# salesforce/gorp

Hardware: AMD Instinct MI355X
Metric: lines/sec (Gorp.extract: product-DFA match + capture offsets; results as narrow rows (int8 id + uint8 offsets, 9 B/line)) (higher is better)
Workload: dtype u8

## Files before the change

### gorp_amd/csrc/gx_api.cpp

```cpp
#include <hip/hip_runtime.h>

#include <algorithm>
#include <array>
#include <cstdio>
#include <cstddef>
#include <cstdlib>
#include <map>
#include <mutex>
#include <new>
#include <optional>
#include <string>
#include <thread>
#include <atomic>

#include "gx_by_key.hpp"
#include "gx_compile.hpp"
#include "gx_device.hpp"
#include "gx_dsl.hpp"
#include "gx_group.hpp"
#include "gx_group_quantile.hpp"
#include "gx_top_groups.hpp"
#include "gx_hop.hpp"
#include "gx_images.hpp"
#include "gx_slots.hpp"
// ... 725 lines not shown
    case 5: { GxLds L; return plan_tile_launch(I, 0, &L) ? static_cast<int64_t>(L.total_bytes) : 0; }
    case 6: { GxLds L; return plan_tile_launch(I, 0, &L) ? static_cast<int64_t>(L.nwaves) : 0; }
    case 7: return !I.tile_ok ? 0 : I.dense[0].L.tier == 3 ? 4 : I.tile_global ? 2 : I.dense[0].L.tier == 2 ? 3 : 1;
    case 8: return h->T.has_capture ? 1 : 0;
    case 10: { GxLds L; return plan_lanes_launch(I, &L, false, true) ? static_cast<int64_t>(L.nwaves) : 0; }
    case 11: { GxLds L; return plan_lanes_launch(I, &L, true, false) ? static_cast<int64_t>(L.nwaves) : 0; }
    case 12: return I.tile_ok ? static_cast<int64_t>(I.dense[0].L.table_bytes) : 0;
    case 13: return I.tile_ok ? static_cast<int64_t>(I.dense[0].L.regs_wave_bytes) : 0;
    case 14: return I.hop[0].ok ? static_cast<int64_t>(H.n_states) : 0;
    case 15: return I.hop[0].ok ? static_cast<int64_t>(H.full.n_hot) : 0;
    case 21: return I.hop[0].ok ? static_cast<int64_t>(H.small.n_hot) : 0;
    case 16: return I.hop[0].ok ? static_cast<int64_t>(H.n_reachable_hot) : 0;
    case 17: return I.hop[0].ok ? static_cast<int64_t>(H.n_chains) : 0;
    case 18: { GxLds L; return plan_hop_launch(I, 0, &L) ? static_cast<int64_t>(L.nwaves) : 0; }
    case 20: return I.hop[0].ok ? static_cast<int64_t>(H.full.n_lds_rows) : 0;
    case 22: return I.hop[1].ok ? static_cast<int64_t>(I.hop[1].img.n_states) : 0;
    case 24: return static_cast<int64_t>(h->slots.promises_broken.load());
    case 30: return static_cast<int64_t>(h->peer_image_bytes);
    case 25: return h->last_kernel.load();
    case 31: return h->last_fits.load();
    case 32: return h->last_limit.load();
    case 33: return static_cast<int64_t>(h->last_utf8_lines.load());
    case 34: return static_cast<int64_t>(h->last_utf8_units.load());
    case 26: return I.hop_reason;
    case 28: return static_cast<int64_t>(h->svc.enabled ? h->svc.launches : -1);
    case 27: { int64_t c = 0; for (auto& r : h->T.rules) c += r.pike ? 1 : 0; return c; }
    case 35: {
        if (!h->T.has_pike()) return -1;
        uint32_t lane_ints = 0, blocks = 0;
        pike_sizing(h->T, &lane_ints, &blocks);
// ... 2792 lines not shown
```

### gorp_amd/csrc/gx_hop.cpp

```cpp
#include "gx_hop.hpp"

#include <algorithm>
#include <deque>

namespace gx {

namespace {
inline bool has(const ClassSet& s, int c) { return (s[c >> 6] >> (c & 63)) & 1ull; }
inline void put(ClassSet& s, int c) { s[c >> 6] |= 1ull << (c & 63); }
}

std::vector<int> order_classes(const std::map<ClassSet, uint64_t>& weight, int ncls) {
    std::vector<std::vector<int>> blocks(1);
    for (int c = 0; c < ncls; ++c) blocks[0].push_back(c);
    std::vector<std::pair<uint64_t, ClassSet>> by_weight;
    for (auto& w : weight) {
        int size = 0;
        for (int c = 0; c < ncls; ++c) size += has(w.first, c) ? 1 : 0;
        if (size > 1 && size < ncls) by_weight.push_back({w.second * static_cast<uint64_t>(size), w.first});
    }
    std::sort(by_weight.begin(), by_weight.end(), [](const std::pair<uint64_t, ClassSet>& a, const std::pair<uint64_t, ClassSet>& b) {
        return a.first != b.first ? a.first > b.first : a.second < b.second;
    });
    for (auto& ws : by_weight) {
// ... 82 lines not shown
        for (int i = 0; i < 128; ++i) {
            if (!in_set(m, i)) continue;
            int j = i;
            long w = 0;
            while (j < 128 && in_set(m, j)) { w += byte_worth(j); ++j; }
            if (w > best.weight || (w == best.weight && j - i > best.hi - best.lo + 1)) best = Range{i, j - 1, w};
            i = j;
        }
        return best;
    };

    struct Exit { bool any = false; Range r; uint32_t entry = 0; ClassSet set{}; };
    std::vector<Range> run(S);
    std::vector<long> run_weight(S, 0);
    std::vector<std::array<uint8_t, 8>> set_table(1, std::array<uint8_t, 8>{0, 0, 0, 0, 0x80, 0x80, 0x80, 0x80});
    std::map<std::array<uint8_t, 8>, uint32_t> set_index;
    std::vector<uint32_t> set_of(S, 0);
    auto loop_set = [&](const ClassSet& cs) -> uint32_t {
        const ByteSet m = bytes_of(cs);
        std::vector<Range> rs;
        for (int i = 0; i < 128; ++i) {
            if (!in_set(m, i)) continue;
            int j = i;
            long w = 0;
            while (j < 128 && in_set(m, j)) { w += byte_worth(j); ++j; }
            rs.push_back(Range{i, j - 1, w});
            i = j;
        }
        if (rs.size() < 2) return 0u;
        std::stable_sort(rs.begin(), rs.end(), [](const Range& a, const Range& b) { return a.weight != b.weight ? a.weight > b.weight : (a.hi - a.lo) > (b.hi - b.lo); });
        if (rs.size() > 4) rs.resize(4);
        std::sort(rs.begin(), rs.end(), [](const Range& a, const Range& b) { return a.lo < b.lo; });
        std::array<uint8_t, 8> key{0, 0, 0, 0, 0x80, 0x80, 0x80, 0x80};
        for (size_t q = 0; q < rs.size(); ++q) { key[q] = static_cast<uint8_t>(rs[q].lo); key[4 + q] = static_cast<uint8_t>(0x7F - rs[q].hi); }
        auto it = set_index.find(key);
        if (it != set_index.end()) return it->second;
        if (set_table.size() >= 256) return 0u;
        set_table.push_back(key);
        set_index[key] = static_cast<uint32_t>(set_table.size() - 1);
        return static_cast<uint32_t>(set_table.size() - 1);
    };
    std::vector<Exit> exit_of(S);
    std::vector<std::vector<uint32_t>> plausible_targets(S);
    for (size_t s = 0; s < S; ++s) {
        int n_plausible = 0;
        const Group* only = nullptr;
        for (auto& g : groups[s]) {
            if (g.entry == static_cast<uint32_t>(s)) {
                run[s] = best_range(g.set);
                run_weight[s] = g.weight;
                if (s != dead) set_of[s] = loop_set(g.set);
                continue;
            }
            if (g.weight > 0) { ++n_plausible; only = &g; plausible_targets[s].push_back(g.entry & 0xFFFFu); }
        }
        if (n_plausible == 1) {
            exit_of[s].any = true;
            exit_of[s].r = best_range(only->set);
            exit_of[s].entry = only->entry;
            exit_of[s].set = only->set;
        }
    }

    struct Chain { int klen = 0, tail = -1; uint8_t lo[HOP_CHAIN], span[HOP_CHAIN]; uint32_t target = 0, col[2] = {0, 0}, off[2] = {0, 0}, tail_set = 0; };
    std::vector<Chain> chain(S);
    for (size_t s = 0; s < S; ++s) {
// ... 4 lines not shown
        for (uint32_t k = 0; k < HOP_CHAIN; ++k) {
            if (k > 0 && run_weight[cur] > 4) break;
            const Exit& x = exit_of[cur];
            if (!x.any || x.r.hi < x.r.lo) break;
            const bool ranged = x.r.hi > x.r.lo || x.r.lo == 0;
            if (ranged && ch.tail >= 0) break;
            const uint32_t col = x.entry >> 16;
            if (col) {
                if (nops == 2) break;
                ch.col[nops] = col;
                ch.off[nops] = k;
                ++nops;
            }
            if (ranged) {
                ch.tail = static_cast<int>(k);
                ch.tail_set = loop_set(x.set);
            }
            ch.lo[k] = static_cast<uint8_t>(x.r.lo);
            ch.span[k] = static_cast<uint8_t>(x.r.hi - x.r.lo);
            ch.klen = static_cast<int>(k) + 1;
            cur = x.entry & 0xFFFFu;
        }
        ch.target = static_cast<uint32_t>(cur);
    }

    std::vector<uint32_t> order;
    std::vector<char> seen(S, 0);
    std::deque<uint32_t> queue;
    auto visit = [&](uint32_t s) { if (!seen[s]) { seen[s] = 1; queue.push_back(s); } };
    visit(0);
    while (!queue.empty()) {
// ... 54 lines not shown
        const Chain& ch = chain[s];
        uint32_t run_lo = 0, run_k = 0x80;
        if (run[s].hi >= run[s].lo && s != dead) { run_lo = static_cast<uint32_t>(run[s].lo); run_k = 0x7Fu - static_cast<uint32_t>(run[s].hi); ++out.n_runs; }
        r[0] = run_lo | run_k << 8 | static_cast<uint32_t>(ch.klen) << 16 | set_of[s] << 24;
        r[1] = (ch.klen ? perm[ch.target] : 0u) | ch.off[0] << 16 | ch.off[1] << 24;
        r[2] = (ch.col[0] << 7) | (ch.col[1] << 7) << 16;
        uint8_t lits[HOP_CHAIN];
        for (uint32_t k = 0; k < HOP_CHAIN; ++k) lits[k] = (static_cast<int>(k) < ch.klen && static_cast<int>(k) != ch.tail) ? ch.lo[k] : 0;
        if (ch.tail >= 0) r[3] = static_cast<uint32_t>(ch.tail) | static_cast<uint32_t>(ch.lo[ch.tail]) << 8 | static_cast<uint32_t>(ch.span[ch.tail]) << 16 | ch.tail_set << 24;
        else r[3] = 0u | 0u << 8 | 0xFFu << 16;
        if (ch.klen == 0) r[3] = 0u | 2u << 8 | 0u << 16, lits[0] = 0x01;
        else ++out.n_chains;
        memcpy(&r[4], lits, 8);
    }

    for (size_t s = 0; s < S; ++s) {
        const uint32_t* r = &hops[s * (HOP_REC_BYTES / 4)];
        const uint32_t run_lo = r[0] & 0xFFu, run_k = (r[0] >> 8) & 0xFFu;
        if (run_k != 0x80u)
            for (uint32_t bt = run_lo; bt <= 0x7Fu - run_k; ++bt)
                if (rows[s * cols + T.cls256[bt]] != static_cast<uint32_t>(s)) throw GxError(GX_E_ARG, "internal: hop tier run does not match the dense rows");
        {
            const std::array<uint8_t, 8>& ls = set_table[r[0] >> 24];
            for (int q = 0; q < 4; ++q)
                if (ls[4 + q] != 0x80u)
                    for (uint32_t bt = ls[q]; bt <= 0x7Fu - ls[4 + q]; ++bt)
                        if (rows[s * cols + T.cls256[bt]] != static_cast<uint32_t>(s)) throw GxError(GX_E_ARG, "internal: hop tier loop set does not match the dense rows");
        }
        const uint32_t klen = (r[0] >> 16) & 0xFFu;
        const uint8_t* lits = reinterpret_cast<const uint8_t*>(&r[4]);
        const uint32_t tail_pos = r[3] & 0xFFu, tail_lo = (r[3] >> 8) & 0xFFu, tail_span = (r[3] >> 16) & 0xFFu;
        uint32_t cur = static_cast<uint32_t>(s), nops = 0;
        const uint32_t want_col[2] = {(r[2] & 0xFFFFu) >> 7, (r[2] >> 16) >> 7}, want_off[2] = {(r[1] >> 16) & 0xFFu, r[1] >> 24};
        if (klen > HOP_CHAIN || tail_pos >= HOP_CHAIN) throw GxError(GX_E_ARG, "internal: hop tier chain length");
        for (uint32_t k = 0; k < klen; ++k) {
            uint32_t lo = lits[k], hi = lits[k];
            if (lits[k] == 0) {
                if (k != tail_pos) throw GxError(GX_E_ARG, "internal: hop tier chain element without a test");
                lo = tail_lo; hi = tail_lo + tail_span;
                const std::array<uint8_t, 8>& ts = set_table[r[3] >> 24];
                for (int q = 0; q < 4; ++q)
                    if (ts[4 + q] != 0x80u)
                        for (uint32_t bt = ts[q]; bt <= 0x7Fu - ts[4 + q]; ++bt)
                            if (rows[cur * cols + T.cls256[bt]] != rows[cur * cols + T.cls256[lo]]) throw GxError(GX_E_ARG, "internal: hop tier chain tail set is not one group");
            } else if (k == tail_pos && (lits[k] < tail_lo || lits[k] > tail_lo + tail_span)) lo = 1, hi = 0;
            if (hi > 0x7Fu) throw GxError(GX_E_ARG, "internal: hop tier chain element out of range");
            if (hi < lo) continue;
            const uint32_t e0 = rows[cur * cols + T.cls256[lo]];
            for (uint32_t bt = lo; bt <= hi; ++bt) if (rows[cur * cols + T.cls256[bt]] != e0) throw GxError(GX_E_ARG, "internal: hop tier chain element is not one group");
            if (e0 >> 16) {
                if (nops >= 2 || want_col[nops] != (e0 >> 16) || want_off[nops] != k) throw GxError(GX_E_ARG, "internal: hop tier chain programs");
                ++nops;
            }
            cur = e0 & 0xFFFFu;
        }
        if (klen && tail_pos >= klen && !(tail_lo == 0 && tail_span == 0xFFu)) throw GxError(GX_E_ARG, "internal: hop tier chain tail beyond the chain");
        if (klen && (cur != (r[1] & 0xFFFFu) || (nops < 2 && want_col[nops] != 0))) throw GxError(GX_E_ARG, "internal: hop tier chain target");
    }

// ... 89 lines not shown
```

### gorp_amd/csrc/gx_hop.hpp

```cpp
#pragma once
#include <array>
#include <map>

#include "gx_compile.hpp"

namespace gx {

typedef std::array<uint64_t, 4> ClassSet;

std::vector<int> order_classes(const std::map<ClassSet, uint64_t>& weight, int ncls);

constexpr uint32_t HOP_REC_BYTES = 24;
constexpr uint32_t HOP_AT = 272;
constexpr uint32_t HOP_CHAIN = 8;

struct HopLds {
    std::vector<uint8_t> bytes;
    uint32_t n_hot = 0, info_lds = 0, fin_lds = 0, n_lds_rows = 0;
    uint32_t sets_lds = 0;
};

struct HopImage {
    bool ok = false;
    uint32_t refused = 0;
    HopLds full;
    HopLds small;
    std::vector<uint8_t> global;
    uint32_t ncls = 0, row_bytes = 0, n_states = 0, n_hot = 0;
    uint32_t hops_off = 0, fin_off = 0;
    uint32_t fin_state_off = 0, fin_state_rec = 0;
    uint32_t start = 0, dead = 0;
    uint32_t n_regs = 0;
    uint32_t col_unset = 0;
    bool match_automaton = false;
    uint32_t n_reachable_hot = 0, n_chains = 0, n_runs = 0, n_loop_sets = 0;
};

bool build_hop_image(const Tables& T, bool match_automaton, uint32_t hot_budget_bytes, uint32_t small_budget_bytes, HopImage& out);

}
```

### gorp_amd/csrc/gx_hop_dev.hpp

```cpp
#pragma once
#include "gx_walk.hpp"

namespace gx {

constexpr uint32_t HOP_REC_B = 24, HOP_LDS_AT = 272, LOW7 = 0x7F7F7F7Fu;

struct HopTab {
    const uint8_t* rows;
    const uint8_t* hops;
    uint32_t row_bytes;
    uint32_t info_off;
    uint32_t n_hot;
    uint32_t lrow_cols;
    uint32_t sets;
};

struct __attribute__((packed, aligned(4))) HopPair { u32x2 v; };
__device__ __forceinline__ u32x2 lds_pair4(uint32_t a) { return ((GX_LDS const HopPair*)(uintptr_t)a)->v; }
__device__ __forceinline__ uint32_t sat_add(uint32_t a, uint32_t b) {
    uint32_t r;
    asm("v_add_u32_e64 %0, %1, %2 clamp" : "=v"(r) : "v"(a), "v"(b));
    return r;
}
__device__ __forceinline__ uint32_t min3u(uint32_t a, uint32_t b, uint32_t c) {
    uint32_t r;
    asm("v_min3_u32 %0, %1, %2, %3" : "=v"(r) : "v"(a), "v"(b), "v"(c));
    return r;
}
__device__ __forceinline__ uint32_t bfi(uint32_t mask, uint32_t a, uint32_t b) {
// ... 19 lines not shown
}

__device__ __forceinline__ bool wave_any(bool c) { return __builtin_amdgcn_ballot_w64(c) != 0ull; }

__device__ __forceinline__ uint32_t run_flags(uint32_t x, uint32_t lo4, uint32_t k4) {
    return (x | (x - lo4) | (x + k4)) & HI_BITS;
}
struct HopKept {
    uint32_t hint = 0u;
#ifdef GX_DEV
    uint32_t dev_iters = 0u, dev_lane_iters = 0u;
#endif
    uint32_t kept = 0xFFFFFFFFu;
    u32x2 k0 = {0u, 0u}, k1 = {0u, 0u}, k2 = {0u, 0u};
};
template <bool ALL_HOT, bool CAPTURE, bool SECOND = true>
__device__ __forceinline__ uint32_t walk_hop_span(const HopTab& H, uint32_t& p, uint32_t e, uint32_t limit, uint32_t e_chain, uint32_t p0,
                                                  uint32_t s, uint32_t dead, uint32_t regs, uint32_t leave_at, HopKept& K) {
    const uint32_t dummy_col = regs - 128u;
    const uint32_t last_hot = H.n_hot - 1u;
    auto exact_step_c = [&](uint32_t lrow, uint32_t c, uint32_t q) {
        uint32_t xe;
        if (lrow) xe = lds_ld<uint16_t>(lrow + (c << 1)) | static_cast<uint32_t>(lds_ld<uint8_t>(lrow + H.lrow_cols + c)) << 16;
        else xe = *reinterpret_cast<const uint32_t*>(H.rows + (static_cast<uint64_t>(s) * H.row_bytes + (c << 2)));
        if (CAPTURE) lds_st<uint16_t>(dummy_col + ((xe >> 16) << 7), static_cast<uint16_t>(q - p0));
        s = xe & 0xFFFFu;
        p = s == dead ? max(limit, q + 1u) : q + 1u;
    };
    auto exact_step = [&](uint32_t lrow, uint32_t bt, uint32_t q) { exact_step_c(lrow, lds_ld<uint8_t>(bt), q); };
    if (ALL_HOT && __builtin_amdgcn_ballot_w64(s > last_hot) != 0ull)
        while (s > last_hot && p < limit) exact_step(0u, lds_ld<uint8_t>(p), p);
// ... 19 lines not shown
            if ((__builtin_amdgcn_ballot_w64(s != kept) & unfinished) != 0ull) {
                if (s != kept && p < limit) {
                    if (s <= last_hot) {
                        const uint32_t la = __umul24(s, HOP_REC_B) + HOP_LDS_AT;
                        k0 = lds_ld<u32x2>(la); k1 = lds_ld<u32x2>(la + 8u); k2 = lds_ld<u32x2>(la + 16u);
                    } else {
                        const u32x2* g = reinterpret_cast<const u32x2*>(H.hops + static_cast<uint64_t>(s) * HOP_REC_B);
                        k0 = g[0]; k1 = g[1]; k2 = g[2];
                    }
                    kept = s;
                }
            }
            h0 = k0; h1 = k1; h2 = k2;
        }
        const uint32_t lo4 = splat_byte0(h0.x), k4 = splat_byte1(h0.x);
        uint32_t wlen, n, q;
        auto run_window = [&]() {
            const uint32_t a1 = p & ~3u, sh1 = p & 3u;
            const u32x2 d01 = lds_pair4(a1), d23 = lds_pair4(a1 + 8u);
            const uint32_t x0 = __builtin_amdgcn_alignbyte(d01.y, d01.x, sh1), x1 = __builtin_amdgcn_alignbyte(d23.x, d01.y, sh1);
            const uint32_t x2 = __builtin_amdgcn_alignbyte(d23.y, d23.x, sh1), x3 = __builtin_amdgcn_alignbyte(0xFFFFFFFFu, d23.y, sh1);
            const uint32_t f0 = static_cast<uint32_t>(__ffs(static_cast<int>(run_flags(x0, lo4, k4))) - 1);
            const uint32_t f1 = static_cast<uint32_t>(__ffs(static_cast<int>(run_flags(x1, lo4, k4))) - 1);
            const uint32_t f2 = static_cast<uint32_t>(__ffs(static_cast<int>(run_flags(x2, lo4, k4))) - 1);
            const uint32_t f3 = static_cast<uint32_t>(__ffs(static_cast<int>(run_flags(x3, lo4, k4))) - 1);
            n = min3u(f0, sat_add(f1, 32u), min3u(sat_add(f2, 64u), sat_add(f3, 96u), 128u)) >> 3;
            n = min(n, e - p);
            wlen = 16u - sh1;
            q = p + n;
        };
        run_window();
        const uint64_t m_step = __builtin_amdgcn_ballot_w64(n < wlen) & __builtin_amdgcn_ballot_w64(q < e) & unfinished;
        const uint32_t a2 = q & ~3u, sh2 = q & 3u;
        const u32x2 r01 = lds_pair4(a2);
        const uint32_t r2 = lds_ld<uint32_t>(a2 + 8u);
        const uint32_t v0 = __builtin_amdgcn_alignbyte(r01.y, r01.x, sh2), v1 = __builtin_amdgcn_alignbyte(r2, r01.y, sh2);
        const uint32_t sad = __builtin_amdgcn_msad_u8(v1, h2.y, __builtin_amdgcn_msad_u8(v0, h2.x, 0u));
        const uint32_t tail = sub_b0_b1(__builtin_amdgcn_perm(v1, v0, h1.y), h1.y);
        const uint32_t qk = add_byte2(q, h0.x);
        const uint32_t span = (h1.y >> 16) & 0xFFu;
        const bool chain_ok = sad == 0u && tail <= span && qk <= e_chain;
        const uint64_t m_chain = m_step & __builtin_amdgcn_ballot_w64(sad == 0u) & __builtin_amdgcn_ballot_w64(tail <= span) & __builtin_amdgcn_ballot_w64(qk <= e_chain);
        const bool stepping = n < wlen && q < e && p < limit;
        const bool chained = stepping && chain_ok;
        const uint32_t cols = chained ? h1.x : 0u;
        const uint32_t rel = q - p0;
        if (CAPTURE) {
            lds_st<uint16_t>(add_word0(dummy_col, cols), static_cast<uint16_t>(add_byte2(rel, h0.y)));
            lds_st<uint16_t>(add_word1(dummy_col, cols), static_cast<uint16_t>(add_byte3(rel, h0.y)));
        }
        p = p < limit ? (chained ? qk : q) : p;
        s = chained ? (h0.y & 0xFFFFu) : s;
        const uint64_t m_exact = m_step & ~m_chain;
        if (m_exact != 0ull) {
            bool exact = stepping && !chained;
            const uint32_t cls_q = lds_ld<uint8_t>(v0 & 0xFFu);
            if (!SECOND) {
                if (__builtin_amdgcn_ballot_w64(exact && ((h0.x | h1.y) >> 24) != 0u) != 0ull) K.hint = 1u;
            } else {
            const u32x2 ts = lds_ld<u32x2>(H.sets + ((h1.y >> 24) << 3)), ls = lds_ld<u32x2>(H.sets + ((h0.x >> 24) << 3));
            if ((__builtin_amdgcn_ballot_w64(sad == 0u && (h1.y >> 24) != 0u && qk <= e_chain) & m_exact) != 0ull) {
                const bool retry = exact && sad == 0u && qk <= e_chain;
                const uint32_t tb = __builtin_amdgcn_perm(v1, v0, h1.y) & 0xFFu;
                if (retry && run_flags(tb * 0x01010101u, ts.x, ts.y) != HI_BITS) {
                    if (CAPTURE) {
                        lds_st<uint16_t>(add_word0(dummy_col, h1.x), static_cast<uint16_t>(add_byte2(rel, h0.y)));
                        lds_st<uint16_t>(add_word1(dummy_col, h1.x), static_cast<uint16_t>(add_byte3(rel, h0.y)));
                    }
                    p = qk;
                    s = h0.y & 0xFFFFu;
                    exact = false;
                }
            }
// ... 11 lines not shown
                nu = min(nu, e - q);
                if (exact && nu != 0u) { p = q + nu; exact = false; }
            }
            if (__builtin_amdgcn_ballot_w64(stepping && !chained && !exact) != 0ull) K.hint = 1u;
            }
            if (exact) {
                exact_step_c(((h0.x >> 16) & 0xFFu) == 0u ? (h0.y & 0xFFFFu) << 2 : 0u, cls_q, q);
                if (ALL_HOT)
                    while (s > last_hot && p < limit) exact_step(0u, lds_ld<uint8_t>(p), p);
            }
        }
    }
    return s;
}

template <bool CAPTURE>
__device__ __forceinline__ uint32_t walk_hop(const HopTab& H, bool all_hot, uint32_t stage, uint32_t s, uint32_t start, uint32_t end, bool on,
                                             uint32_t dead, uint32_t regs, bool& second) {
    const uint32_t p0 = stage + start, e = stage + end;
    uint32_t p = on ? p0 : e;
    HopKept K;
    uint32_t r;
    if (all_hot) r = second ? walk_hop_span<true, CAPTURE, true>(H, p, e, e, e, p0, s, dead, regs, 0u, K) : walk_hop_span<true, CAPTURE, false>(H, p, e, e, e, p0, s, dead, regs, 0u, K);
    else r = walk_hop_span<false, CAPTURE, true>(H, p, e, e, e, p0, s, dead, regs, 0u, K);
    second = K.hint != 0u;
    return r;
}

}
```

### gorp_amd/csrc/gx_images.cpp

```cpp
#include "gx_images.hpp"

#include <array>
#include <cstdio>
#include <cstdlib>
#include <map>

namespace gx {

namespace {

template <typename F> uint16_t self_loop_interval(F loops) {
    int best_lo = 0, best_len = 0, run_lo = 0, run = 0;
    for (int b = 0; b < 128; ++b) {
        if (loops(b)) { if (run == 0) run_lo = b; ++run; if (run >= best_len) { best_len = run; best_lo = run_lo; } }
        else run = 0;
    }
    if (best_len < 4) return 0x8000;
    return static_cast<uint16_t>(best_lo | ((0x7F - (best_lo + best_len - 1)) << 8));
}

constexpr uint32_t REC_MORE = 0x80u << 24, REC_HDR = 2u << 24, REC_IDC = 254u, REC_EMPTY = 255u, REC_AT = 1088u;

bool records_from_dense(const Tables& T, const std::vector<uint32_t>& at, size_t rows, uint32_t cols, const std::vector<uint32_t>& dead_of_row,
                        const std::vector<std::array<uint64_t, 2>>& loop_set, bool simple, Image& img, GxLds& L, std::vector<uint32_t>& c_rule,
// ... 579 lines not shown
        L.m_start = M.match_automaton ? M.start : 0u;
        L.m_dead = M.match_automaton ? M.dead : 0u;
        L.u_start = M.match_automaton ? 0xFFFFFFFFu : M.start;
        L.u_dead = M.match_automaton ? 0xFFFFFFFFu : M.dead;
        L.fin_tags = M.fin_off;
        L.fin_state_off = M.fin_state_off;
        L.fin_state_rec = M.fin_state_rec;
        L.simple_ops = 1;
        L.tier = 4;
        L.rec = HOP_AT;
        L.sort_chunk = M.n_reachable_hot;
        L.hot_lo4 = 0;
        L.hot_k4 = 0x80808080u;
        L.regs_wave_bytes = static_cast<uint32_t>(((M.n_regs + 1) * 64 * 2 + 15) & ~15u);
        L.fin_unset = M.col_unset;
        for (int q = 0; q < 2; ++q) {
            const HopLds& P = q ? M.small : M.full;
            L.table_bytes = static_cast<uint32_t>(P.bytes.size());
            L.rec_indexed = P.n_hot;
            L.acc_tab = P.info_lds;
            L.at = P.fin_lds;
            L.hop_sets = P.sets_lds;
            (q ? H.small : H.full) = L;
        }
        GxLds P;
        H.ok = plan_tile_layout(H.full, 200, &P);
    };
    I.hop_reason = 4;
    if (!no_tiles && want_hop && T.has_capture && !(flags & GX_CREATE_NO_FUSED)) {
        hop_tier(false);
// ... 61 lines not shown
```

### gorp_amd/csrc/gx_kernels.hip

```cpp
#include "gx_rows.hpp"
#include "gx_hop_dev.hpp"

namespace gx {

namespace {

constexpr int GENERIC_MAX_REGS = 96;

template <typename CH>
__device__ __forceinline__ int class_of(const GxDev& T, CH ch) {
    uint32_t c = static_cast<uint32_t>(ch);
    if (sizeof(CH) == 1 || c < 256u) return T.cls256[c];
    int lo = 0, hi = T.n_hi;
    while (hi - lo > 1) {
        int mid = (lo + hi) >> 1;
        if (T.hi_lo[mid] <= c) lo = mid; else hi = mid;
    }
    return T.hi_cls[lo];
}

template <typename CH>
__device__ bool pike_capture(const GxDev& T, int k, const CH* __restrict__ s, int64_t len, int32_t* __restrict__ scratch, int32_t* __restrict__ caps_out) {
    const uint32_t base = T.pike_off[k], n_inst = T.pike_off[k + 1] - base;
    const uint32_t* code = T.pike_code + 2ull * base;
// ... 506 lines not shown
    unsigned long long ph[6] = {0, 0, 0, 0, 0, 0}, ph_t = __builtin_amdgcn_s_memtime();
    unsigned long long dv[6] = {0, 0, 0, 0, 0, 0};
    const unsigned long long hs_begin = __builtin_amdgcn_s_memrealtime();
#define HS_STAMP(slot) do { const unsigned long long now_ = __builtin_amdgcn_s_memtime(); ph[slot] += now_ - ph_t; ph_t = now_; } while (0)
#else
#define HS_STAMP(slot) do { } while (0)
#endif
    HopTab H;
    H.rows = at_global;
    H.hops = at_global + L.c_base;
    H.row_bytes = L.row_bytes;
    H.info_off = L.ncls * 4u;
    H.n_hot = L.rec_indexed;
    H.lrow_cols = (2u * L.ncls + 3u) & ~3u;
    H.sets = L.hop_sets;
    const uint32_t lane = threadIdx.x & 63u;
    const uint32_t wave = threadIdx.x >> 6;
    const uint32_t slice = L.stage + wave * L.stage_bytes;
    const uint32_t regs = L.regs + wave * L.regs_wave_bytes + 128u + lane * 2u;
    const uint8_t* data_end = data + (static_cast<uint64_t>(off[n]) << (WIDE ? 1 : 0));
    const uint32_t row0 = match_only ? L.m_start : L.u_start, dead_row = match_only ? L.m_dead : L.u_dead;
    const uint8_t* fin_g = L.at != 0u ? nullptr : at_global + L.fin_tags;
    const uint32_t fin_lds = L.at;

    const uint64_t nwaves = static_cast<uint64_t>(gridDim.x) * L.nwaves;
    const uint64_t per_wave = (n_static + nwaves - 1) / nwaves;
    const uint64_t wid = static_cast<uint64_t>(blockIdx.x) * L.nwaves + wave;
    const uint64_t range_lo = min(n_static, wid * per_wave);
    uint64_t range_hi = min(n_static, range_lo + per_wave);
    uint64_t next = range_lo;
// ... 419 lines not shown
```

### gorp_amd/csrc/gx_layout.hpp

```cpp
#pragma once
#include <cstdint>

namespace gx {

constexpr uint32_t LDS_BYTES = 163840;
constexpr uint32_t LDS_TABLE_BUDGET = 96 * 1024;

struct GxLds {
    uint32_t cmap;
    uint32_t ncls;
    uint32_t at;
    uint32_t row_bytes;
    uint32_t c_base;
    uint32_t m_start;
    uint32_t m_dead;
    uint32_t c_rule;
    uint32_t u_start;
    uint32_t u_dead;
    uint32_t ops_off;
    uint32_t ops;
    uint32_t fin_tags;
    uint32_t table_bytes;
    uint32_t simple_ops;
    uint32_t regs;
    uint32_t regs_wave_bytes;
    uint32_t bitmap;
    uint32_t counter;
    uint32_t stage;
    uint32_t stage_bytes;
    uint32_t nwaves;
    uint32_t total_bytes;
    uint32_t hot_lo4, hot_k4;
    uint32_t tier;
    uint32_t rec, acc_tab;
    uint32_t rec_indexed;
    uint32_t sort_lds;
    uint32_t sort_chunk;
    uint32_t hop_sets;
    uint32_t fin_unset;
    uint32_t fin_state_off, fin_state_rec;
};
constexpr uint32_t GX_STEAL_MAX = 3072;
constexpr uint32_t GX_STEAL_STRIDE = 32;
constexpr uint32_t GX_BITMAP_WAVE_BYTES = 144;

#ifndef GX_HOP_SLICE_BYTES
#define GX_HOP_SLICE_BYTES 128u
#endif
constexpr uint32_t GX_SERVICE_MAX_BYTES = 56u + 16u * 60u;

enum RowFormat : uint32_t { ROWS_DENSE = 0, ROWS_U16 = 1, ROWS_U8 = 2 };
constexpr RowFormat row_format(bool compact, bool narrow) { return !compact ? ROWS_DENSE : narrow ? ROWS_U8 : ROWS_U16; }
constexpr uint32_t row_unit_bytes(RowFormat f) { return f == ROWS_U8 ? 1u : f == ROWS_U16 ? 2u : 4u; }
// ... 16 lines not shown
```

### gorp_amd/csrc/gx_tile_body.hpp

```cpp
#pragma once
#include "gx_rows.hpp"
#include "gx_hop_dev.hpp"

namespace gx {

namespace {

struct TileIO {
    const uint8_t* image;
    const uint8_t* at_global;
    const uint8_t* data;
    const void* off;
    uint64_t n;
    RowOut rows;
    uint32_t* oversize_flag;
    uint32_t seq;
    int32_t max_groups;
    int32_t strip_eol;
    uint32_t* steal;
    uint32_t steal_parity;
    uint32_t share64;
    uint8_t* wide_flags;
    uint32_t* wide_any;
    int32_t* state_out;
// ... 174 lines not shown
        for (uint32_t q = blockIdx.x * blockDim.x + threadIdx.x; q < GX_STEAL_MAX; q += gridDim.x * blockDim.x) other[q * GX_STEAL_STRIDE] = 0u;
        if (threadIdx.x == 0) lds_st<uint32_t>(L.counter, 0u);
    }
    __syncthreads();

    constexpr bool GT = TIER == TIER_L2 || TIER == TIER_RECG || TIER == TIER_HOP;
    constexpr bool HOP = TIER == TIER_HOP;
    HopTab H;
    H.rows = io.at_global;
    H.hops = io.at_global + L.c_base;
    H.row_bytes = L.row_bytes;
    H.info_off = L.ncls * 4u;
    H.n_hot = L.rec_indexed;
    H.lrow_cols = (2u * L.ncls + 3u) & ~3u;
    H.sets = L.hop_sets;
    const uint8_t* __restrict__ data = io.data;
    const OFF* __restrict__ off = static_cast<const OFF*>(io.off);
    const uint64_t n = io.n;
    WalkTab Wm, Wc;
    Wm.at = GT ? io.at_global + (TIER == TIER_RECG ? L.c_base : 0u) : nullptr;
    Wm.row_bytes = L.row_bytes;
    Wm.ops_off = L.ops_off;
    Wm.ops = L.ops;
    Wm.acc_tab = L.acc_tab;
    Wm.ncls = L.ncls;
    Wm.indexed = L.rec_indexed;
    Wc = Wm;
    if (GT) Wc.at = io.at_global + L.c_base;

    const uint32_t lane = threadIdx.x & 63u;
// ... 133 lines not shown
    uint64_t tile = tile_at(blockIdx.x, wave);
    uint64_t t1 = tile_at(blockIdx.x, L.nwaves + wave);
    uint64_t t2 = tiles;
    uint32_t g3 = 0, jn = 0u, gn = 0u;
    bool sh3 = false, shn = false;
    uint32_t j3 = draw_ticket(1u);
    sh3 = draw_shared(j3, 1u, g3);
    bool need_t2 = true, stealing = false, drew_before = false;
    if (tile >= tiles) return;
#ifdef GX_DEV
    unsigned long long phase_cycles[4] = {0, 0, 0, 0};
    unsigned long long stamp_ = __builtin_amdgcn_s_memtime();
    const unsigned long long dev_begin = __builtin_amdgcn_s_memrealtime();
    unsigned long long dev_tiles = 0;
#endif
    bool hop_second = false;
    u32x4 pre[WIDE ? 2 * KCH : KCH];
    uint64_t no0 = 0, no1 = 0;
    TileInfo cur;
    {
        uint64_t o0, o1;
        load_offsets(tile, o0, o1);
        cur = make_round(tile, 0, o0, o1);
    }
    load_offsets(min(t1, tiles - 1), no0, no1);
    tile_issue_loads<KCH, WIDE>(cur, lane, pre, io.image);

    for (;;) {
        const bool wide_line = tile_commit<KCH, HOP, WIDE>(cur, lane, pre, stage, bitmap, use_map, L.hot_lo4, L.hot_k4, data, data_end);
        GX_STAMP(0);
        const uint32_t group_lines = static_cast<uint32_t>(min(static_cast<uint64_t>(64), n - (tile << 6)));
// ... 25 lines not shown
        shn = draw_shared(jn, drew ? 1u : 0u, gn);
        drew_before = drew;
        GX_STAMP(1);

        const uint64_t i = cur.i;
        const bool valid = cur.active != 0u;
        const uint32_t start = cur.start;
        uint32_t end = cur.end;
        if (io.strip_eol && cur.mode != 2) {
            if (end > start && lds_ld<uint8_t>(stage + end - 1u) == 0x0Au) --end;
            if (end > start && lds_ld<uint8_t>(stage + end - 1u) == 0x0Du) --end;
        }
        if (cur.mode == 2) {
            if (lane == cur.a) announce_left_line(io.oversize_flag, io.seq);
        } else if (MODE == 0 && HOP) {
            const uint32_t mrow = walk_hop<false>(H, L.rec_indexed >= L.sort_chunk, stage, L.m_start, start, end, true, L.m_dead, regs, hop_second);
            int32_t first = static_cast<int16_t>(lds_ld<uint16_t>(L.acc_tab + 2u * min(mrow, H.n_hot - 1u)));
            if (wave_any(mrow >= H.n_hot)) {
                if (mrow >= H.n_hot) first = *reinterpret_cast<const int32_t*>(H.rows + (static_cast<uint64_t>(mrow) * H.row_bytes + H.info_off));
            }
            if (valid) io.rows.match_id[i] = first;
            GX_STAMP(2);
        } else if (MODE == 0) {
            const uint32_t mrow = walk<TIER, false, false>(Wm, stage, bitmap, use_map, L.m_start, start, end, true, L.m_dead, regs);
            if (valid) io.rows.match_id[i] = state_info<TIER>(Wm, mrow);
            if ((TIER == TIER_LDS || TIER == TIER_L2) && io.state_out && valid)
                io.state_out[i] = mrow == L.m_dead ? -1 : static_cast<int32_t>(TIER == TIER_LDS ? (mrow - L.m_start) / L.row_bytes : mrow - L.m_start);
            GX_STAMP(2);
        } else {
            int32_t info;
            if (HOP) {
                const uint32_t urow = walk_hop<true>(H, L.rec_indexed >= L.sort_chunk, stage, L.u_start, start, end, true, L.u_dead, regs, hop_second);
                const int32_t hot_info = static_cast<int16_t>(lds_ld<uint16_t>(L.acc_tab + 2u * min(urow, H.n_hot - 1u)));
                info = hot_info >= 0 ? hot_info * 16 : hot_info;
                if (wave_any(urow >= H.n_hot)) {
                    if (urow >= H.n_hot) info = *reinterpret_cast<const int32_t*>(H.rows + (static_cast<uint64_t>(urow) * H.row_bytes + H.info_off));
                }
            } else if (MODE == 1 || L.u_start != 0xFFFFFFFFu) {
                uint32_t urow;
                if (MODE == 1 || L.simple_ops) urow = walk<TIER, true, true>(Wc, stage, bitmap, use_map, L.u_start, start, end, true, L.u_dead, regs);
                else urow = walk<TIER, true, false>(Wc, stage, bitmap, use_map, L.u_start, start, end, true, L.u_dead, regs);
                info = state_info<TIER>(Wc, urow);
            } else {
                const uint32_t mrow = walk<TIER, false, false>(Wm, stage, bitmap, use_map, L.m_start, start, end, true, L.m_dead, regs);
                const int32_t k = state_info<TIER>(Wm, mrow);
                info = k;
                uint32_t crow = GT ? 0u : L.m_dead;
// ... 108 lines not shown
```

Baseline: 28.18 billion.

## Widen hop-tier run tests with case-fold and digit flags, adaptive wide mode

The host image builder now tags each loop set and chain tail with flags saying the state also self-loops, or exits alike, on the opposite-case letters or on digits. Those flags are packed into a per-image bitmask, and the device run and tail tests can then accept such bytes in one SIMD compare instead of stopping for an exact per-byte step. Device use is adaptive: the cheap kernel counts how many exact steps hit set-bearing records, and past a threshold the next block of tiles runs the wide variant. This replaces the earlier boolean second-pass switch. The cost is extra ALU work per window while the wide variant is active, plus host-side validation work.

```diff
diff --git a/gorp_amd/csrc/gx_api.cpp b/gorp_amd/csrc/gx_api.cpp
--- a/gorp_amd/csrc/gx_api.cpp
+++ b/gorp_amd/csrc/gx_api.cpp
@@ -763,6 +763,9 @@
     case 17: return I.hop[0].ok ? static_cast<int64_t>(H.n_chains) : 0;
     case 18: { GxLds L; return plan_hop_launch(I, 0, &L) ? static_cast<int64_t>(L.nwaves) : 0; }
     case 20: return I.hop[0].ok ? static_cast<int64_t>(H.full.n_lds_rows) : 0;
+    case 36: return I.hop[0].ok ? static_cast<int64_t>(H.n_fold) : 0;
+    case 37: return I.hop[0].ok ? static_cast<int64_t>(H.n_digits) : 0;
+    case 38: return I.hop[0].ok ? static_cast<int64_t>(H.wide_sets) : 0;
     case 22: return I.hop[1].ok ? static_cast<int64_t>(I.hop[1].img.n_states) : 0;
     case 24: return static_cast<int64_t>(h->slots.promises_broken.load());
     case 30: return static_cast<int64_t>(h->peer_image_bytes);
diff --git a/gorp_amd/csrc/gx_hop.cpp b/gorp_amd/csrc/gx_hop.cpp
--- a/gorp_amd/csrc/gx_hop.cpp
+++ b/gorp_amd/csrc/gx_hop.cpp
@@ -120,9 +120,10 @@
     std::vector<Range> run(S);
     std::vector<long> run_weight(S, 0);
     std::vector<std::array<uint8_t, 8>> set_table(1, std::array<uint8_t, 8>{0, 0, 0, 0, 0x80, 0x80, 0x80, 0x80});
-    std::map<std::array<uint8_t, 8>, uint32_t> set_index;
+    std::map<std::pair<std::array<uint8_t, 8>, uint32_t>, uint32_t> set_index;
+    std::vector<uint32_t> set_flags(1, 0u);
     std::vector<uint32_t> set_of(S, 0);
-    auto loop_set = [&](const ClassSet& cs) -> uint32_t {
+    auto loop_set = [&](const ClassSet& cs, uint32_t flags) -> uint32_t {
         const ByteSet m = bytes_of(cs);
         std::vector<Range> rs;
         for (int i = 0; i < 128; ++i) {
@@ -139,12 +140,18 @@
         std::sort(rs.begin(), rs.end(), [](const Range& a, const Range& b) { return a.lo < b.lo; });
         std::array<uint8_t, 8> key{0, 0, 0, 0, 0x80, 0x80, 0x80, 0x80};
         for (size_t q = 0; q < rs.size(); ++q) { key[q] = static_cast<uint8_t>(rs[q].lo); key[4 + q] = static_cast<uint8_t>(0x7F - rs[q].hi); }
-        auto it = set_index.find(key);
+        if (flags && set_index.find({key, flags}) == set_index.end() && set_table.size() >= HOP_WIDE_SETS) flags = 0u;
+        auto it = set_index.find({key, flags});
         if (it != set_index.end()) return it->second;
         if (set_table.size() >= 256) return 0u;
         set_table.push_back(key);
-        set_index[key] = static_cast<uint32_t>(set_table.size() - 1);
+        set_flags.push_back(flags);
+        set_index[{key, flags}] = static_cast<uint32_t>(set_table.size() - 1);
         return static_cast<uint32_t>(set_table.size() - 1);
+    };
+    auto loops_plainly = [&](size_t s, int lo, int hi) {
+        for (int bt = lo; bt <= hi; ++bt) if (ent[s * ncls + T.cls256[bt]] != static_cast<uint32_t>(s)) return false;
+        return true;
     };
     std::vector<Exit> exit_of(S);
     std::vector<std::vector<uint32_t>> plausible_targets(S);
@@ -155,7 +162,14 @@
             if (g.entry == static_cast<uint32_t>(s)) {
                 run[s] = best_range(g.set);
                 run_weight[s] = g.weight;
-                if (s != dead) set_of[s] = loop_set(g.set);
+                if (s != dead) {
+                    uint32_t flags = 0u;
+                    if (run[s].hi >= run[s].lo) {
+                        if (run[s].lo >= 'a' && run[s].hi <= 'z' && loops_plainly(s, run[s].lo ^ 0x20, run[s].hi ^ 0x20)) flags |= HOP_FOLD;
+                        if (((run[s].lo >= 'a' && run[s].hi <= 'z') || (run[s].lo >= '0' && run[s].hi <= '9')) && loops_plainly(s, '0', '9')) flags |= HOP_DIGITS;
+                    }
+                    set_of[s] = loop_set(g.set, flags);
+                }
                 continue;
             }
             if (g.weight > 0) { ++n_plausible; only = &g; plausible_targets[s].push_back(g.entry & 0xFFFFu); }
@@ -190,7 +204,14 @@
             }
             if (ranged) {
                 ch.tail = static_cast<int>(k);
-                ch.tail_set = loop_set(x.set);
+                uint32_t flags = 0u;
+                auto exits_alike = [&](int lo, int hi) {
+                    for (int bt = lo; bt <= hi; ++bt) if (ent[cur * ncls + T.cls256[bt]] != x.entry) return false;
+                    return true;
+                };
+                if (x.r.lo >= 'a' && x.r.hi <= 'z' && exits_alike(x.r.lo ^ 0x20, x.r.hi ^ 0x20)) flags |= HOP_FOLD;
+                if (((x.r.lo >= 'a' && x.r.hi <= 'z') || (x.r.lo >= '0' && x.r.hi <= '9')) && exits_alike('0', '9')) flags |= HOP_DIGITS;
+                ch.tail_set = loop_set(x.set, flags);
             }
             ch.lo[k] = static_cast<uint8_t>(x.r.lo);
             ch.span[k] = static_cast<uint8_t>(x.r.hi - x.r.lo);
@@ -275,12 +296,28 @@
         memcpy(&r[4], lits, 8);
     }
 
+    uint32_t wide_sets = 0;
+    for (size_t q = 1; q < set_table.size() && q < HOP_WIDE_SETS; ++q) wide_sets |= ((set_flags[q] & HOP_FOLD) ? 1u << q : 0u) | ((set_flags[q] & HOP_DIGITS) ? 0x10000u << q : 0u);
+    out.wide_sets = wide_sets;
+
     for (size_t s = 0; s < S; ++s) {
         const uint32_t* r = &hops[s * (HOP_REC_BYTES / 4)];
         const uint32_t run_lo = r[0] & 0xFFu, run_k = (r[0] >> 8) & 0xFFu;
         if (run_k != 0x80u)
             for (uint32_t bt = run_lo; bt <= 0x7Fu - run_k; ++bt)
                 if (rows[s * cols + T.cls256[bt]] != static_cast<uint32_t>(s)) throw GxError(GX_E_ARG, "internal: hop tier run does not match the dense rows");
+        const uint32_t wide = (r[0] >> 24) < HOP_WIDE_SETS ? wide_sets >> (r[0] >> 24) : 0u;
+        if (wide & 1u) {
+            if (run_k == 0x80u || run_lo < 'a' || 0x7Fu - run_k > 'z') throw GxError(GX_E_ARG, "internal: hop tier fold flag on a run outside a-z");
+            for (uint32_t bt = 0; bt < 0x80u; ++bt)
+                if ((bt | 0x20u) >= run_lo && (bt | 0x20u) <= 0x7Fu - run_k && rows[s * cols + T.cls256[bt]] != static_cast<uint32_t>(s)) throw GxError(GX_E_ARG, "internal: hop tier fold flag does not match the dense rows");
+            ++out.n_fold;
+        }
+        if (wide & 0x10000u) {
+            for (uint32_t bt = '0'; bt <= '9'; ++bt)
+                if (rows[s * cols + T.cls256[bt]] != static_cast<uint32_t>(s)) throw GxError(GX_E_ARG, "internal: hop tier digits flag does not match the dense rows");
+            ++out.n_digits;
+        }
         {
             const std::array<uint8_t, 8>& ls = set_table[r[0] >> 24];
             for (int q = 0; q < 4; ++q)
@@ -304,6 +341,12 @@
                     if (ts[4 + q] != 0x80u)
                         for (uint32_t bt = ts[q]; bt <= 0x7Fu - ts[4 + q]; ++bt)
                             if (rows[cur * cols + T.cls256[bt]] != rows[cur * cols + T.cls256[lo]]) throw GxError(GX_E_ARG, "internal: hop tier chain tail set is not one group");
+                const uint32_t tw = (r[3] >> 24) < HOP_WIDE_SETS ? wide_sets >> (r[3] >> 24) : 0u;
+                if ((tw & 1u) && (lo < 'a' || hi > 'z')) throw GxError(GX_E_ARG, "internal: hop tier fold flag on a tail outside a-z");
+                for (uint32_t bt = 0; bt < 0x80u; ++bt) {
+                    const bool let = ((tw & 1u) && (bt | 0x20u) >= lo && (bt | 0x20u) <= hi) || ((tw & 0x10000u) && bt >= '0' && bt <= '9');
+                    if (let && rows[cur * cols + T.cls256[bt]] != rows[cur * cols + T.cls256[lo]]) throw GxError(GX_E_ARG, "internal: hop tier chain tail flags do not match the dense rows");
+                }
             } else if (k == tail_pos && (lits[k] < tail_lo || lits[k] > tail_lo + tail_span)) lo = 1, hi = 0;
             if (hi > 0x7Fu) throw GxError(GX_E_ARG, "internal: hop tier chain element out of range");
             if (hi < lo) continue;
diff --git a/gorp_amd/csrc/gx_hop.hpp b/gorp_amd/csrc/gx_hop.hpp
--- a/gorp_amd/csrc/gx_hop.hpp
+++ b/gorp_amd/csrc/gx_hop.hpp
@@ -13,6 +13,7 @@
 constexpr uint32_t HOP_REC_BYTES = 24;
 constexpr uint32_t HOP_AT = 272;
 constexpr uint32_t HOP_CHAIN = 8;
+constexpr uint32_t HOP_FOLD = 1u, HOP_DIGITS = 2u, HOP_WIDE_SETS = 16;
 
 struct HopLds {
     std::vector<uint8_t> bytes;
@@ -33,7 +34,8 @@
     uint32_t n_regs = 0;
     uint32_t col_unset = 0;
     bool match_automaton = false;
-    uint32_t n_reachable_hot = 0, n_chains = 0, n_runs = 0, n_loop_sets = 0;
+    uint32_t n_reachable_hot = 0, n_chains = 0, n_runs = 0, n_loop_sets = 0, n_fold = 0, n_digits = 0;
+    uint32_t wide_sets = 0;
 };
 
 bool build_hop_image(const Tables& T, bool match_automaton, uint32_t hot_budget_bytes, uint32_t small_budget_bytes, HopImage& out);
diff --git a/gorp_amd/csrc/gx_hop_dev.hpp b/gorp_amd/csrc/gx_hop_dev.hpp
--- a/gorp_amd/csrc/gx_hop_dev.hpp
+++ b/gorp_amd/csrc/gx_hop_dev.hpp
@@ -13,6 +13,7 @@
     uint32_t n_hot;
     uint32_t lrow_cols;
     uint32_t sets;
+    uint32_t wide;
 };
 
 struct __attribute__((packed, aligned(4))) HopPair { u32x2 v; };
@@ -62,7 +63,7 @@
     uint32_t kept = 0xFFFFFFFFu;
     u32x2 k0 = {0u, 0u}, k1 = {0u, 0u}, k2 = {0u, 0u};
 };
-template <bool ALL_HOT, bool CAPTURE, bool SECOND = true>
+template <bool ALL_HOT, bool CAPTURE, bool SECOND = true, bool WIDE_RUN = false>
 __device__ __forceinline__ uint32_t walk_hop_span(const HopTab& H, uint32_t& p, uint32_t e, uint32_t limit, uint32_t e_chain, uint32_t p0,
                                                   uint32_t s, uint32_t dead, uint32_t regs, uint32_t leave_at, HopKept& K) {
     const uint32_t dummy_col = regs - 128u;
@@ -112,16 +113,28 @@
             h0 = k0; h1 = k1; h2 = k2;
         }
         const uint32_t lo4 = splat_byte0(h0.x), k4 = splat_byte1(h0.x);
+        uint32_t fold4 = 0u, dlo4 = 0u, dk4 = HI_BITS;
+        if (WIDE_RUN) {
+            const uint32_t w = H.wide >> min(h0.x >> 24, 16u);
+            fold4 = static_cast<uint32_t>(__builtin_amdgcn_sbfe(static_cast<int>(w), 0u, 1u)) & 0x20202020u;
+            const uint32_t dm = static_cast<uint32_t>(__builtin_amdgcn_sbfe(static_cast<int>(w), 16u, 1u));
+            dlo4 = dm & 0x30303030u;
+            dk4 = bfi(dm, 0x46464646u, HI_BITS);
+        }
+        auto run_test = [&](uint32_t x) {
+            if (!WIDE_RUN) return run_flags(x, lo4, k4);
+            return run_flags(x | fold4, lo4, k4) & run_flags(x, dlo4, dk4);
+        };
         uint32_t wlen, n, q;
         auto run_window = [&]() {
             const uint32_t a1 = p & ~3u, sh1 = p & 3u;
             const u32x2 d01 = lds_pair4(a1), d23 = lds_pair4(a1 + 8u);
             const uint32_t x0 = __builtin_amdgcn_alignbyte(d01.y, d01.x, sh1), x1 = __builtin_amdgcn_alignbyte(d23.x, d01.y, sh1);
             const uint32_t x2 = __builtin_amdgcn_alignbyte(d23.y, d23.x, sh1), x3 = __builtin_amdgcn_alignbyte(0xFFFFFFFFu, d23.y, sh1);
-            const uint32_t f0 = static_cast<uint32_t>(__ffs(static_cast<int>(run_flags(x0, lo4, k4))) - 1);
-            const uint32_t f1 = static_cast<uint32_t>(__ffs(static_cast<int>(run_flags(x1, lo4, k4))) - 1);
-            const uint32_t f2 = static_cast<uint32_t>(__ffs(static_cast<int>(run_flags(x2, lo4, k4))) - 1);
-            const uint32_t f3 = static_cast<uint32_t>(__ffs(static_cast<int>(run_flags(x3, lo4, k4))) - 1);
+            const uint32_t f0 = static_cast<uint32_t>(__ffs(static_cast<int>(run_test(x0))) - 1);
+            const uint32_t f1 = static_cast<uint32_t>(__ffs(static_cast<int>(run_test(x1))) - 1);
+            const uint32_t f2 = static_cast<uint32_t>(__ffs(static_cast<int>(run_test(x2))) - 1);
+            const uint32_t f3 = static_cast<uint32_t>(__ffs(static_cast<int>(run_test(x3))) - 1);
             n = min3u(f0, sat_add(f1, 32u), min3u(sat_add(f2, 64u), sat_add(f3, 96u), 128u)) >> 3;
             n = min(n, e - p);
             wlen = 16u - sh1;
@@ -134,11 +147,18 @@
         const uint32_t r2 = lds_ld<uint32_t>(a2 + 8u);
         const uint32_t v0 = __builtin_amdgcn_alignbyte(r01.y, r01.x, sh2), v1 = __builtin_amdgcn_alignbyte(r2, r01.y, sh2);
         const uint32_t sad = __builtin_amdgcn_msad_u8(v1, h2.y, __builtin_amdgcn_msad_u8(v0, h2.x, 0u));
-        const uint32_t tail = sub_b0_b1(__builtin_amdgcn_perm(v1, v0, h1.y), h1.y);
+        const uint32_t tbytes = __builtin_amdgcn_perm(v1, v0, h1.y);
         const uint32_t qk = add_byte2(q, h0.x);
         const uint32_t span = (h1.y >> 16) & 0xFFu;
-        const bool chain_ok = sad == 0u && tail <= span && qk <= e_chain;
-        const uint64_t m_chain = m_step & __builtin_amdgcn_ballot_w64(sad == 0u) & __builtin_amdgcn_ballot_w64(tail <= span) & __builtin_amdgcn_ballot_w64(qk <= e_chain);
+        bool tail_ok;
+        if (WIDE_RUN) {
+            const uint32_t tw = H.wide >> min(h1.y >> 24, 16u);
+            const uint32_t tfold = static_cast<uint32_t>(__builtin_amdgcn_sbfe(static_cast<int>(tw), 0u, 1u)) & 0x20u;
+            const uint32_t tdigits = (tw >> 16) & 1u;
+            tail_ok = sub_b0_b1(tbytes | tfold, h1.y) <= span || sub_b0_b1(tbytes, 0x3000u) < tdigits * 10u;
+        } else tail_ok = sub_b0_b1(tbytes, h1.y) <= span;
+        const bool chain_ok = sad == 0u && tail_ok && qk <= e_chain;
+        const uint64_t m_chain = m_step & __builtin_amdgcn_ballot_w64(sad == 0u) & __builtin_amdgcn_ballot_w64(tail_ok) & __builtin_amdgcn_ballot_w64(qk <= e_chain);
         const bool stepping = n < wlen && q < e && p < limit;
         const bool chained = stepping && chain_ok;
         const uint32_t cols = chained ? h1.x : 0u;
@@ -154,7 +174,7 @@
             bool exact = stepping && !chained;
             const uint32_t cls_q = lds_ld<uint8_t>(v0 & 0xFFu);
             if (!SECOND) {
-                if (__builtin_amdgcn_ballot_w64(exact && ((h0.x | h1.y) >> 24) != 0u) != 0ull) K.hint = 1u;
+                K.hint += static_cast<uint32_t>(__builtin_popcountll(__builtin_amdgcn_ballot_w64(exact && ((h0.x | h1.y) >> 24) != 0u)));
             } else {
             const u32x2 ts = lds_ld<u32x2>(H.sets + ((h1.y >> 24) << 3)), ls = lds_ld<u32x2>(H.sets + ((h0.x >> 24) << 3));
             if ((__builtin_amdgcn_ballot_w64(sad == 0u && (h1.y >> 24) != 0u && qk <= e_chain) & m_exact) != 0ull) {
@@ -196,17 +216,23 @@
     return s;
 }
 
+constexpr uint32_t HOP_WIDE_TILES = 63u, HOP_WIDE_WANTED = 64u;
 template <bool CAPTURE>
 __device__ __forceinline__ uint32_t walk_hop(const HopTab& H, bool all_hot, uint32_t stage, uint32_t s, uint32_t start, uint32_t end, bool on,
-                                             uint32_t dead, uint32_t regs, bool& second) {
+                                             uint32_t dead, uint32_t regs, uint32_t& wide_left) {
     const uint32_t p0 = stage + start, e = stage + end;
     uint32_t p = on ? p0 : e;
     HopKept K;
     uint32_t r;
-    if (all_hot) r = second ? walk_hop_span<true, CAPTURE, true>(H, p, e, e, e, p0, s, dead, regs, 0u, K) : walk_hop_span<true, CAPTURE, false>(H, p, e, e, e, p0, s, dead, regs, 0u, K);
-    else r = walk_hop_span<false, CAPTURE, true>(H, p, e, e, e, p0, s, dead, regs, 0u, K);
-    second = K.hint != 0u;
-    return r;
-}
-
-}
+    if (!all_hot) r = walk_hop_span<false, CAPTURE, true>(H, p, e, e, e, p0, s, dead, regs, 0u, K);
+    else if (wide_left != 0u) {
+        r = walk_hop_span<true, CAPTURE, true, true>(H, p, e, e, e, p0, s, dead, regs, 0u, K);
+        --wide_left;
+    } else {
+        r = walk_hop_span<true, CAPTURE, false>(H, p, e, e, e, p0, s, dead, regs, 0u, K);
+        if (K.hint >= HOP_WIDE_WANTED) wide_left = HOP_WIDE_TILES;
+    }
+    return r;
+}
+
+}
diff --git a/gorp_amd/csrc/gx_images.cpp b/gorp_amd/csrc/gx_images.cpp
--- a/gorp_amd/csrc/gx_images.cpp
+++ b/gorp_amd/csrc/gx_images.cpp
@@ -617,6 +617,7 @@
         L.hot_k4 = 0x80808080u;
         L.regs_wave_bytes = static_cast<uint32_t>(((M.n_regs + 1) * 64 * 2 + 15) & ~15u);
         L.fin_unset = M.col_unset;
+        L.hop_wide = M.wide_sets;
         for (int q = 0; q < 2; ++q) {
             const HopLds& P = q ? M.small : M.full;
             L.table_bytes = static_cast<uint32_t>(P.bytes.size());
diff --git a/gorp_amd/csrc/gx_kernels.hip b/gorp_amd/csrc/gx_kernels.hip
--- a/gorp_amd/csrc/gx_kernels.hip
+++ b/gorp_amd/csrc/gx_kernels.hip
@@ -544,6 +544,7 @@
     H.n_hot = L.rec_indexed;
     H.lrow_cols = (2u * L.ncls + 3u) & ~3u;
     H.sets = L.hop_sets;
+    H.wide = L.hop_wide;
     const uint32_t lane = threadIdx.x & 63u;
     const uint32_t wave = threadIdx.x >> 6;
     const uint32_t slice = L.stage + wave * L.stage_bytes;
diff --git a/gorp_amd/csrc/gx_layout.hpp b/gorp_amd/csrc/gx_layout.hpp
--- a/gorp_amd/csrc/gx_layout.hpp
+++ b/gorp_amd/csrc/gx_layout.hpp
@@ -37,6 +37,7 @@
     uint32_t sort_lds;
     uint32_t sort_chunk;
     uint32_t hop_sets;
+    uint32_t hop_wide;
     uint32_t fin_unset;
     uint32_t fin_state_off, fin_state_rec;
 };
diff --git a/gorp_amd/csrc/gx_tile_body.hpp b/gorp_amd/csrc/gx_tile_body.hpp
--- a/gorp_amd/csrc/gx_tile_body.hpp
+++ b/gorp_amd/csrc/gx_tile_body.hpp
@@ -212,6 +212,7 @@
     H.n_hot = L.rec_indexed;
     H.lrow_cols = (2u * L.ncls + 3u) & ~3u;
     H.sets = L.hop_sets;
+    H.wide = L.hop_wide;
     const uint8_t* __restrict__ data = io.data;
     const OFF* __restrict__ off = static_cast<const OFF*>(io.off);
     const uint64_t n = io.n;
@@ -375,7 +376,7 @@
     const unsigned long long dev_begin = __builtin_amdgcn_s_memrealtime();
     unsigned long long dev_tiles = 0;
 #endif
-    bool hop_second = false;
+    uint32_t hop_wide_left = 0u;
     u32x4 pre[WIDE ? 2 * KCH : KCH];
     uint64_t no0 = 0, no1 = 0;
     TileInfo cur;
@@ -431,7 +432,7 @@
         if (cur.mode == 2) {
             if (lane == cur.a) announce_left_line(io.oversize_flag, io.seq);
         } else if (MODE == 0 && HOP) {
-            const uint32_t mrow = walk_hop<false>(H, L.rec_indexed >= L.sort_chunk, stage, L.m_start, start, end, true, L.m_dead, regs, hop_second);
+            const uint32_t mrow = walk_hop<false>(H, L.rec_indexed >= L.sort_chunk, stage, L.m_start, start, end, true, L.m_dead, regs, hop_wide_left);
             int32_t first = static_cast<int16_t>(lds_ld<uint16_t>(L.acc_tab + 2u * min(mrow, H.n_hot - 1u)));
             if (wave_any(mrow >= H.n_hot)) {
                 if (mrow >= H.n_hot) first = *reinterpret_cast<const int32_t*>(H.rows + (static_cast<uint64_t>(mrow) * H.row_bytes + H.info_off));
@@ -447,7 +448,7 @@
         } else {
             int32_t info;
             if (HOP) {
-                const uint32_t urow = walk_hop<true>(H, L.rec_indexed >= L.sort_chunk, stage, L.u_start, start, end, true, L.u_dead, regs, hop_second);
+                const uint32_t urow = walk_hop<true>(H, L.rec_indexed >= L.sort_chunk, stage, L.u_start, start, end, true, L.u_dead, regs, hop_wide_left);
                 const int32_t hot_info = static_cast<int16_t>(lds_ld<uint16_t>(L.acc_tab + 2u * min(urow, H.n_hot - 1u)));
                 info = hot_info >= 0 ? hot_info * 16 : hot_info;
                 if (wave_any(urow >= H.n_hot)) {
```

Result: no change. 28.18 billion, median of 6 (-0.0%).
